# HiKapok/DAN

Hardware: AMD Instinct MI355X
Metric: 640x640 images/sec/node (train fwd+bwd) (higher is better)
Workload: dtype bf16; 1 GPU; S3FD VGG-16 backbone + 6 detection heads, 640x640 bf16 training (fwd+bwd+SGD), batch 16 per GPU; global_batch=16, parallelism=dp1, anchors_per_image=34125, step_launch=eager, rccl_ranks=1, weight_gradient_stream=True

## Files before the change

dan_amd/_lib.py:

```python
import ctypes
import os

import torch

_HERE = os.path.dirname(os.path.abspath(__file__))
ACT_NAME = os.environ.get("DANHIP_DTYPE", "bf16").lower()
if ACT_NAME not in ("bf16", "fp16"):
    raise ValueError("DANHIP_DTYPE must be bf16 or fp16, got %r" % ACT_NAME)
ACT_DTYPE = torch.float16 if ACT_NAME == "fp16" else torch.bfloat16
SO_PATH = os.path.join(_HERE, "libdanhip_f16.so" if ACT_NAME == "fp16" else "libdanhip.so")
if os.environ.get("DANHIP_LIB_PATH"):
    SO_PATH = os.path.abspath(os.environ["DANHIP_LIB_PATH"])

F32, BF16 = 0, 1
SPLIT3 = 3


class ConvDesc(ctypes.Structure):
    _fields_ = [(n, ctypes.c_int32) for n in ("N", "H", "W", "Cin", "Ho", "Wo", "Cout", "kh", "kw", "stride")]


class ConvPitch(ctypes.Structure):
    _fields_ = [(n, ctypes.c_int32) for n in ("x_pitch", "y_pitch", "aux_pitch")]


class PackEntry(ctypes.Structure):
    _fields_ = [("w_hwio", ctypes.c_void_p), ("wf_packed", ctypes.c_void_p), ("wb_packed", ctypes.c_void_p)] + \
               [(n, ctypes.c_int32) for n in ("kh", "kw", "cin", "cin_real", "cout", "rows_f", "cols_f", "rows_b", "cols_b", "co8", "first_block", "pad_")]


class JpegInfo(ctypes.Structure):
    _fields_ = [(n, ctypes.c_int32) for n in ("width", "height", "ncomp", "mode", "reason", "reserved")] + [("coef_count", ctypes.c_int64)]


class JpegDesc(ctypes.Structure):
    _fields_ = [(n, ctypes.c_int32) for n in ("width", "height", "ncomp", "mode")] + \
               [(n, ctypes.c_int32 * 3) for n in ("blocks_w", "blocks_h", "comp_w", "comp_h", "quant_index")] + \
               [(n, ctypes.c_int32) for n in ("status", "idct_groups", "rgb_groups")] + [("reserved", ctypes.c_int32 * 2)] + \
               [("coef_offset", ctypes.c_int64), ("coef_count", ctypes.c_int64), ("plane_offset", ctypes.c_int64 * 3),
                ("out_offset", ctypes.c_int64), ("quant", (ctypes.c_uint16 * 64) * 4)]


P = ctypes.c_void_p
I32 = ctypes.c_int32
I64 = ctypes.c_int64
FL = ctypes.c_float
DESC = ctypes.POINTER(ConvDesc)

SIGNATURES = {
    "danhip_conv_packed_dims": [DESC, ctypes.c_int, ctypes.POINTER(I64), ctypes.POINTER(I64)],
    "danhip_pack_conv_weight": [DESC, P, I32, P, P, P],
# ... 57 lines not shown
    "danhip_nms": [P, I32, I32, I32, FL, P, P, P],
    "danhip_argsort_desc_f32": [P, I64, I32, P, P, ctypes.c_size_t, P],
    "danhip_augment_preprocess": [P, I32, I32, I32, ctypes.POINTER(ctypes.c_int32), ctypes.POINTER(ctypes.c_float), I32, I32, I32, I32, I32, P, I32, I32,
                                  P, ctypes.c_size_t, P],
    "danhip_deform_psroi_pool_fwd": [P, P, P, P, P, I32, I32, I32, I32, I32, I32, I32, I32, I32, FL, FL, I32, I32, P],
    "danhip_deform_psroi_pool_bwd": [P, P, P, P, P, P, P, I32, I32, I32, I32, I32, I32, I32, I32, I32, I32, FL, FL, I32, I32, P],
    "danhip_maxpool3x3s2_same_fwd": [P, P, I32, I32, I32, I32, P],
    "danhip_maxpool3x3s2_same_bwd": [P, P, P, I32, I32, I32, I32, P],
    "danhip_resize_u8_linear": [P, I32, I32, P, I32, I32, I32, ctypes.c_double, ctypes.c_double, P],
    "danhip_bbox_vote": [P, P, I32, I32, ctypes.c_double, I32, P, P, P, ctypes.c_size_t, P],
    "danhip_wider_quantize": [P, ctypes.c_int, P, P, I32, I32, I32, P, P, I32, I32, P, P],
    "danhip_wider_score_range": [P, I64, P, P, ctypes.c_size_t, P],
    "danhip_wider_eval": [P, P, I64, P, P, P, I64, P, I32, I32, I32, I32, ctypes.c_double, P, ctypes.c_size_t, P, P],
    "danhip_wider_ap": [P, ctypes.c_size_t, P, I64, I32, I32, I32, P, P, P, P, P, P],
    "danhip_deform_sample_fwd": [P, P, P, I32, I32, I32, I32, I32, I32, I32, I32, I32, P],
    "danhip_deform_sample_bwd": [P, P, P, P, P, I32, I32, I32, I32, I32, I32, I32, I32, I32, ctypes.c_int, P, ctypes.c_size_t, P],
    "danhip_deform_conv_fwd": [P, P, P, P, P, I32, I32, I32, I32, I32, I32, I32, I32, I32, I32, ctypes.c_int, P, ctypes.c_size_t, P],
    "danhip_deform_conv_bwd": [P, P, P, P, P, P, P, P, I32, I32, I32, I32, I32, I32, I32, I32, I32, I32, ctypes.c_int, P, ctypes.c_size_t, P],
    "danhip_deform_conv_bwd_with_col": [P, P, P, P, P, P, P, P, P, I32, I32, I32, I32, I32, I32, I32, I32, I32, I32, ctypes.c_int, P, ctypes.c_size_t, P],
    "danhip_deform_conv_bwd_deliver": [P, P, P, P, P, P, P, P, P, I32, I32, I32, I32, I32, I32, I32, I32, I32, I32, ctypes.c_int, ctypes.c_int, P, ctypes.c_size_t, P],
    "danhip_cast_pad_f32_to_bf16": [P, P, P, I64, I32, I32, P],
    "danhip_head_split_fwd": [P, P, P, I32, I32, I32, I32, I32, I32, I32, P],
    "danhip_head_split_bwd": [P, P, P, P, I32, I32, I32, I32, I32, I32, I32, P],
    "danhip_hard_neg_select": [P, P, P, P, P, P, I32, I32, FL, ctypes.c_int, P],
    "danhip_detection_loss_fwd": [P, P, P, P, P, P, P, P, I32, I32, P],
    "danhip_detection_loss_bwd": [P, P, P, P, P, P, P, FL, FL, I32, I32, P],
    "danhip_sgd_momentum_flat": [P, P, P, P, P, P, I32, I64, FL, FL, FL, P, P],
    "danhip_sgd_momentum_flat_dynamic": [P, P, P, P, P, P, I32, I64, FL, FL, P, P, P],
    "danhip_anchors_generate": [P, P, P, P, P, P, I32, I32, I32, FL, FL, FL, I32, P],
    "danhip_iou_matrix": [P, P, P, P, P, P, P, I32, I32, P],
    "danhip_dual_max_match": [P, I32, I32, FL, FL, ctypes.c_int, P, P, P, ctypes.c_size_t, P],
    "danhip_small_mining_match": [P, I32, I32, FL, FL, FL, I32, FL, P, P, P, ctypes.c_size_t, P],
    "danhip_encode_anchors": [P, P, P, P, P, P, P, P, P, I32, FL, FL, FL, FL, FL, P],
    "danhip_decode_anchors": [P, P, P, P, P, P, I32, I32, FL, FL, FL, FL, P],
    "danhip_face_scores": [P, P, P, FL, I64, P],
    "danhip_comm_load": [ctypes.c_char_p],
    "danhip_comm_rccl_version": [ctypes.POINTER(ctypes.c_int)],
    "danhip_comm_unique_id": [P],
    "danhip_comm_create": [P, I32, I32, I32, ctypes.POINTER(ctypes.c_void_p)],
    "danhip_comm_destroy": [P],
    "danhip_comm_info": [P, ctypes.POINTER(I32), ctypes.POINTER(I32), ctypes.POINTER(I32)],
    "danhip_comm_async_error": [P, ctypes.POINTER(I32)],
    "danhip_comm_abort": [P],
    "danhip_comm_allreduce_sum": [P, P, I64, ctypes.c_int, P],
    "danhip_comm_reduce_scatter_sum": [P, P, P, I64, ctypes.c_int, P],
    "danhip_comm_allgather": [P, P, P, I64, ctypes.c_int, P],
# ... 139 lines not shown
```

dan_amd/csrc/capi.cpp:

```cpp
#include <cstdarg>
#include <cstdio>
#include <cstdlib>
#include <cstring>
#include <atomic>
#include <mutex>

#include <hip/hip_runtime.h>

#include "../../include/danhip.h"

static thread_local char g_err[512] = "";

void danhip_set_error(const char* fmt, ...) {
  va_list ap;
  va_start(ap, fmt);
  vsnprintf(g_err, sizeof(g_err), fmt, ap);
  va_end(ap);
}

extern "C" const char* danhip_last_error(void) { return g_err; }
extern "C" int danhip_version(void) { return 8; }
extern "C" int danhip_act_dtype(void) {
#ifdef DANHIP_FP16
  return DANHIP_F16;
#else
  return DANHIP_BF16;
#endif
}

namespace {
struct Opt { const char* name; const char* env; int def; std::atomic<int> value; };
Opt g_opts[] = {{"splitk", "DANHIP_SPLITK", 1, {0}}, {"wgrad_slab", "DANHIP_WGRAD_SLAB", 1, {0}}, {"halo_b2", "DANHIP_HALO_B2", 0, {0}},
                {"wgrad_b2", "DANHIP_WGRAD_B2", 0, {0}}, {"halo_general_epilogue", "DANHIP_HALO_GENERAL_EPILOGUE", 0, {0}},
                {"deform_bwd_form", "DANHIP_DEFORM_BWD_FORM", 0, {0}}, {"pw_dgrad_ld_bn", "DANHIP_PW_DGRAD_LD_BN", 128, {0}},
                {"wgrad_c8", "DANHIP_WGRAD_C8", 1, {0}}, {"deform_dx_untiled", "DANHIP_DEFORM_DX_UNTILED", 0, {0}}};
std::once_flag g_opts_once;
Opt* find_opt(const char* name) {
  std::call_once(g_opts_once, [] {
    for (Opt& o : g_opts) { const char* e = getenv(o.env); o.value.store(e ? atoi(e) : o.def, std::memory_order_relaxed); }
  });
  if (!name) return nullptr;
  for (Opt& o : g_opts)
    if (strcmp(o.name, name) == 0) return &o;
  return nullptr;
// ... 25 lines not shown
```

dan_amd/csrc/loss.hip:

```cpp
#include "common.h"

namespace {

__device__ __forceinline__ float block_sum(float v, float* sh) {
#pragma unroll
  for (int o = 32; o > 0; o >>= 1) v += __shfl_xor(v, o, 64);
  const int w = threadIdx.x >> 6, nw = blockDim.x >> 6;
  if ((threadIdx.x & 63) == 0) sh[w] = v;
  __syncthreads();
  float t = 0.f;
  for (int i = 0; i < nw; ++i) t += sh[i];
  __syncthreads();
  return t;
}

__global__ void head_split_fwd_kernel(const float* __restrict__ h, float* __restrict__ loc, float* __restrict__ cls, int B, int HW, int Ch,
                                      int nneg, int npos, int A, int off) {
  const long total = (long)B * HW;
  for (long m = (long)blockIdx.x * blockDim.x + threadIdx.x; m < total; m += (long)gridDim.x * blockDim.x) {
    const int b = (int)(m / HW), p = (int)(m % HW);
    const float* r = h + m * Ch;
    const long a = (long)b * A + off + p;
    *reinterpret_cast<float4*>(loc + a * 4) = make_float4(r[0], r[1], r[2], r[3]);
    float ng = r[4];
// ... 5 lines not shown
}

__global__ void head_split_bwd_kernel(const float* __restrict__ h, const float* __restrict__ dloc, const float* __restrict__ dcls,
                                      float* __restrict__ dy, int B, int HW, int Ch, int nneg, int npos, int A, int off) {
  const long total = (long)B * HW;
  for (long m = (long)blockIdx.x * blockDim.x + threadIdx.x; m < total; m += (long)gridDim.x * blockDim.x) {
    const int b = (int)(m / HW), p = (int)(m % HW);
    const float* r = h + m * Ch;
    const long a = (long)b * A + off + p;
    float* o = dy + m * Ch;
    for (int i = 0; i < 4; ++i) o[i] = dloc[a * 4 + i];
    for (int grp = 0; grp < 2; ++grp) {
      const int s = grp == 0 ? 4 : 4 + nneg, n = grp == 0 ? nneg : npos;
      float mx = r[s];
      for (int i = 1; i < n; ++i) mx = fmaxf(mx, r[s + i]);
      int cnt = 0;
      for (int i = 0; i < n; ++i) cnt += (r[s + i] == mx);
      const float g = dcls[a * 2 + grp] / (float)cnt;
      for (int i = 0; i < n; ++i) o[s + i] = r[s + i] == mx ? g : 0.f;
    }
  }
}

__global__ void hard_neg_scores_kernel(const float* __restrict__ cls, const int* __restrict__ labels, float* __restrict__ score,
                                       int* __restrict__ counts, int A) {
  __shared__ int sp, sn;
  if (threadIdx.x == 0) { sp = 0; sn = 0; }
  __syncthreads();
  const int b = blockIdx.y;
  int np = 0, nn = 0;
  for (int a = blockIdx.x * blockDim.x + threadIdx.x; a < A; a += gridDim.x * blockDim.x) {
    const long i = (long)b * A + a;
    const float2 l = *reinterpret_cast<const float2*>(cls + i * 2);
    const float mx = fmaxf(l.x, l.y);
    const float e0 = expf(l.x - mx), e1 = expf(l.y - mx);
    const float pbg = e0 / (e0 + e1);
    const int lab = labels[i];
    score[i] = lab == 0 ? 0.f - pbg : -1.f;
    np += lab > 0;
    nn += lab == 0;
  }
  atomicAdd(&sp, np);
  atomicAdd(&sn, nn);
  __syncthreads();
  if (threadIdx.x == 0) { atomicAdd(counts + b * 2, sp); atomicAdd(counts + b * 2 + 1, sn); }
}
// ... 200 lines not shown

extern "C" int danhip_head_split_fwd(const float* h, float* loc, float* cls, int32_t B, int32_t HW, int32_t Ch, int32_t nneg, int32_t npos,
                                     int32_t A, int32_t anchor_offset, void* stream) {
  DH_REQUIRE(h && loc && cls && B > 0 && HW > 0 && nneg >= 1 && npos >= 1 && Ch == 4 + nneg + npos, DANHIP_EINVAL,
             "head_split_fwd: bad arguments (Ch must be 4+nneg+npos, depth 1)");
  DH_REQUIRE(anchor_offset >= 0 && anchor_offset + HW <= A, DANHIP_EINVAL, "head_split_fwd: anchor range out of bounds");
  hipLaunchKernelGGL(head_split_fwd_kernel, dim3(grid_for((long)B * HW, 256)), dim3(256), 0, (hipStream_t)stream, h, loc, cls, B, HW, Ch, nneg,
                     npos, A, anchor_offset);
  DH_LAUNCH_CHECK();
  return DANHIP_OK;
}

extern "C" int danhip_head_split_bwd(const float* h, const float* dloc, const float* dcls, float* dy, int32_t B, int32_t HW, int32_t Ch,
                                     int32_t nneg, int32_t npos, int32_t A, int32_t anchor_offset, void* stream) {
  DH_REQUIRE(h && dloc && dcls && dy && B > 0 && HW > 0 && nneg >= 1 && npos >= 1 && Ch == 4 + nneg + npos, DANHIP_EINVAL,
             "head_split_bwd: bad arguments");
  DH_REQUIRE(anchor_offset >= 0 && anchor_offset + HW <= A, DANHIP_EINVAL, "head_split_bwd: anchor range out of bounds");
  hipLaunchKernelGGL(head_split_bwd_kernel, dim3(grid_for((long)B * HW, 256)), dim3(256), 0, (hipStream_t)stream, h, dloc, dcls, dy, B, HW, Ch,
                     nneg, npos, A, anchor_offset);
  DH_LAUNCH_CHECK();
  return DANHIP_OK;
}

extern "C" int danhip_hard_neg_select(const float* cls, const int32_t* labels, float* score, int32_t* counts, float* thr, int32_t* k_out,
                                      int32_t B, int32_t A, float negative_ratio, int at_least_one, void* stream) {
  DH_REQUIRE(cls && labels && score && counts && thr && k_out && B > 0 && A > 0, DANHIP_EINVAL, "hard_neg_select: bad arguments");
  hipStream_t s = (hipStream_t)stream;
  if (hipMemsetAsync(counts, 0, sizeof(int32_t) * 2 * B, s) != hipSuccess) { danhip_set_error("hard_neg_select: memset failed"); return DANHIP_ELAUNCH; }
  hipLaunchKernelGGL(hard_neg_scores_kernel, dim3((unsigned)grid_for(A, 1024, 8), (unsigned)B), dim3(1024), 0, s, cls, labels, score, counts, A);
  DH_LAUNCH_CHECK();
  if (A <= 36 * 1024)
    hipLaunchKernelGGL(kth_largest_rows_kernel<36>, dim3((unsigned)B), dim3(1024), 0, s, score, counts, thr, k_out, A, negative_ratio, at_least_one);
  else if (A <= 88 * 1024)
    hipLaunchKernelGGL(kth_largest_rows_kernel<88>, dim3((unsigned)B), dim3(1024), 0, s, score, counts, thr, k_out, A, negative_ratio, at_least_one);
  else
    hipLaunchKernelGGL(kth_largest_rows_kernel<0>, dim3((unsigned)B), dim3(1024), 0, s, score, counts, thr, k_out, A, negative_ratio, at_least_one);
  DH_LAUNCH_CHECK();
  return DANHIP_OK;
}

extern "C" int danhip_detection_loss_fwd(const float* cls, const float* loc, const int32_t* labels, const float* loc_targets, const float* score,
                                         const float* thr, uint8_t* sel, float* acc4, int32_t B, int32_t A, void* stream) {
  DH_REQUIRE(cls && loc && labels && loc_targets && score && thr && sel && acc4 && B > 0 && A > 0, DANHIP_EINVAL, "detection_loss_fwd: bad arguments");
  hipStream_t s = (hipStream_t)stream;
  if (hipMemsetAsync(acc4, 0, sizeof(float) * 4, s) != hipSuccess) { danhip_set_error("detection_loss_fwd: memset failed"); return DANHIP_ELAUNCH; }
  const long total = (long)B * A;
// ... 44 lines not shown
```

dan_amd/net/sfd_net.py:

```python
import os

import torch

from .. import ops
from .variables import VariableStore


POOL_ONLY = os.environ.get("DANHIP_POOL_ONLY", "1") == "1"


class VGG16Backbone(object):
    def __init__(self, data_format="channels_last", bn_epsilon=1e-5, bn_momentum=0.997, use_fused_bn=True, variables=None):
        if data_format != "channels_last":
            raise ValueError("the MI355X build is NHWC-native: use data_format='channels_last' "
                             "(the reference's eval scripts' default, eval_sfd.py:63)")
        self._data_format = data_format
        self._bn_epsilon = bn_epsilon
        self._bn_momentum = bn_momentum
        self._use_fused_bn = use_fused_bn
        self.vs = variables if variables is not None else VariableStore()

    def l2_normalize(self, inputs, init_value, training, name=None):
        w = self.vs.get((name or "l2_normalize") + "/weight", (inputs.shape[-1],), init_value)
        return ops.l2_normalize(inputs, w)
# ... 52 lines not shown
        inputs = self.conv_block(inputs, 2, 128, (3, 3), (1, 1), "conv2", pool_after=True, pool_only=POOL_ONLY)
        inputs = ops.max_pool_2x2(inputs)
        inputs = self.conv_block(inputs, 3, 256, (3, 3), (1, 1), "conv3", pool_after=True)
        feature_layers.append(self.l2_normalize(tap(inputs), 10, training, "l2_norm_layer_3"))
        inputs = ops.max_pool_2x2(inputs)
        inputs = self.conv_block(inputs, 3, 512, (3, 3), (1, 1), "conv4", pool_after=True)
        feature_layers.append(self.l2_normalize(tap(inputs), 8, training, "l2_norm_layer_4"))
        inputs = ops.max_pool_2x2(inputs)
        inputs = self.conv_block(inputs, 3, 512, (3, 3), (1, 1), "conv5", pool_after=True)
        feature_layers.append(self.l2_normalize(tap(inputs), 5, training, "l2_norm_layer_5"))
        inputs = ops.max_pool_2x2(inputs)
        inputs = self.conv_relu(inputs, 1024, (3, 3), (1, 1), "fc6")
        inputs = self.conv_relu(inputs, 1024, (1, 1), (1, 1), "fc7")
        feature_layers.append(tap(inputs))
        inputs = self.conv_relu(inputs, 256, (1, 1), (1, 1), "additional_layers/conv6_1")
        inputs = self.conv_relu(inputs, 512, (3, 3), (2, 2), "additional_layers/conv6_2")
        feature_layers.append(tap(inputs))
        inputs = self.conv_relu(inputs, 128, (1, 1), (1, 1), "additional_layers/conv7_1")
        inputs = self.conv_relu(inputs, 256, (3, 3), (2, 2), "additional_layers/conv7_2")
        feature_layers.append(tap(inputs))
        return feature_layers

    def predict_heads(self, feature_layers, pos_maxout, neg_maxout, num_anchors_depth_per_layer, name, shared_conv=False):
        B = feature_layers[0].shape[0]
        assert all(d == 1 for d in num_anchors_depth_per_layer), "one anchor per cell (all reference configs)"
        A = sum(f.shape[1] * f.shape[2] for f in feature_layers)
        dev = feature_layers[0].device
        loc = torch.zeros((B, A, 4), dtype=torch.float32, device=dev)
        cls = torch.zeros((B, A, 2), dtype=torch.float32, device=dev)
        off = 0
        for ind, feat in enumerate(feature_layers):
            if shared_conv:
                feat = self.conv_relu(feat, feat.shape[-1], (3, 3), (1, 1), "{}/shared_conv_{}".format(name, ind))
            c = feat.shape[-1]
            ncls = pos_maxout[ind] + neg_maxout[ind]
            wl = self.vs.get("{}/loc_{}/kernel".format(name, ind), (3, 3, c, 4), "glorot")
            bl = self.vs.get("{}/loc_{}/bias".format(name, ind), (4,), "zeros")
            wc = self.vs.get("{}/cls_{}/kernel".format(name, ind), (3, 3, c, ncls), "glorot")
            bc = self.vs.get("{}/cls_{}/bias".format(name, ind), (ncls,), "zeros")
            pre = "{}/loc_{}/".format(name, ind), "{}/cls_{}/".format(name, ind)
            wf = self.vs.fuse((pre[0] + "kernel", pre[1] + "kernel"), axis=3)
            bf = self.vs.fuse((pre[0] + "bias", pre[1] + "bias"), axis=0)
            if wf is None or bf is None:
                wf, bf = ops.cat_static([wl, wc], 3), ops.cat_static([bl, bc], 0)
            h = ops.conv2d(feat, wf, bf, stride=1, relu=False, out_f32=True)
            if ops.TRACE is not None and ncls > 2:
                ops.TRACE.setdefault("maxout", {})[id(wc)] = h.detach()[..., 4:]
            loc, cls = ops.head_split(h, loc, cls, neg_maxout[ind], pos_maxout[ind], off)
            off += feat.shape[1] * feat.shape[2]
        return loc, cls

    def multibox_head(self, feature_layers, pos_maxout, neg_maxout, num_anchors_depth_per_layer):
        return self.predict_heads(feature_layers, pos_maxout, neg_maxout, num_anchors_depth_per_layer, "multibox_head")


import contextlib


@contextlib.contextmanager
def precision_scope(precision):
    ctx = ops.context()
    prev = ctx.SPLIT_EVAL
    ctx.SPLIT_EVAL = precision == "split"
    if precision == "split":
        ops.split_range_reset()
    try:
        yield
    finally:
        ctx.SPLIT_EVAL = prev
    if precision == "split":
        ops.split_range_check()


# ... 7 lines not shown
```

dan_amd/ops.py:

```python
import contextlib
import ctypes
import os

import torch

from . import _lib
from ._lib import ACT_DTYPE as ACT, BF16, F32, SPLIT3, ConvDesc, call, ptr, stream


class OpsContext(object):
    __slots__ = ("USE_SPLITK", "USE_SLOTS", "USE_RELU_BITS", "USE_POOL_ARG", "USE_JUNCTION", "POOL_ONLY_TRAIN", "KEEP_DEFORM_COL", "WGRAD_STREAM", "WGRAD_FIRST", "FUSE_FIRST_WGRAD", "SPLIT_EVAL", "TRACE",
                 "PROFILE", "PROFILE_BYTES", "GRAD_READY_HOOK", "LOSS_SCALE_DEV", "wgrad")

    def __init__(self, **overrides):
        env = os.environ.get
        self.USE_SPLITK = True
        self.USE_SLOTS = True
        self.USE_RELU_BITS = env("DANHIP_RELU_BITS", "1") == "1"
        self.USE_POOL_ARG = env("DANHIP_POOL_ARG", "1") == "1"
        self.USE_JUNCTION = env("DANHIP_JUNCTION", "1") == "1"
        self.POOL_ONLY_TRAIN = env("DANHIP_POOL_ONLY_TRAIN", "1") == "1"
        self.KEEP_DEFORM_COL = True
        self.WGRAD_STREAM = env("DANHIP_WGRAD_STREAM", "1") == "1"
        self.WGRAD_FIRST = env("DANHIP_WGRAD_FIRST", "0") == "1"
        self.FUSE_FIRST_WGRAD = env("DANHIP_FUSE_FIRST_WGRAD", "1") == "1"
        self.SPLIT_EVAL = False
        self.TRACE = self.PROFILE = self.PROFILE_BYTES = None
        self.GRAD_READY_HOOK = self.LOSS_SCALE_DEV = None
        self.wgrad = {"on": False, "side": None, "main": None, "keep": []}
        for k, v in overrides.items():
            setattr(self, k, v)


_CTX = OpsContext()
_CTX_FIELDS = frozenset(OpsContext.__slots__) - {"wgrad"}


def context():
    return _CTX


@contextlib.contextmanager
def use_context(ctx):
    global _CTX
    prev, _CTX = _CTX, ctx
    try:
        yield ctx
    finally:
# ... 331 lines not shown
                parg = _pool_arg_buffer(pooled, need_bwd and tracked)
                pool_out.extend([pooled, parg])
            call("danhip_conv2d_fwd_relu_bits_arg", ctypes.byref(d), ptr(x), ptr(wf), ptr(b.detach()), yp, ptr(ybits), ptr(pooled), ptr(pbits), ptr(parg),
                 stream())
            bits_out.extend([ybits, pbits])
        elif pool_out is not None:
            assert relu and not out_f32 and residual is None and b is not None and cout % 8 == 0
            pooled = torch.empty((N, (d.Ho + 1) // 2, (d.Wo + 1) // 2, cout), dtype=ACT, device=x.device)
            parg = _pool_arg_buffer(pooled, need_bwd and tracked)
            ws, nws = _conv_scratch(d, 0, x.device)
            if nws:
                assert not skip_y
                call("danhip_conv2d_fwd_ws", ctypes.byref(d), ptr(x), ptr(wf), ptr(b.detach()), ptr(y), BF16, 1, None, ptr(ws), nws, stream())
                call("danhip_maxpool2x2_fwd_arg", ptr(y), ptr(pooled), ptr(parg), N, d.Ho, d.Wo, cout, stream())
            else:
                call("danhip_conv2d_fwd_pool_arg", ctypes.byref(d), ptr(x), ptr(wf), ptr(b.detach()), yp, ptr(pooled), ptr(parg), stream())
            pool_out.extend([pooled, parg])
        else:
            ws, nws = _conv_scratch(d, 0, x.device)
            call("danhip_conv2d_fwd_ws", ctypes.byref(d), ptr(x), ptr(wf), ptr(b.detach()) if b is not None else None, ptr(y),
                 F32 if out_f32 else BF16, int(relu), ptr(residual), ptr(ws), nws, stream())
        _prof_end(e0, d, 4 if pool_out is not None else 0, wrote_y=not skip_y, pooled=pool_out is not None)
        ctx.d, ctx.relu, ctx.cin_real = d, relu, cin_real
        ctx.xslot, ctx.yslot, ctx.xbits = xslot, yslot, xbits
        ctx.set_materialize_grads(False)
        ctx.has_res = residual is not None
        ctx.w_param, ctx.b_param = w_param, b_param
        ctx.save_for_backward(x, wb, y if (relu and not skip_y) else None)
        ctx.y_unwritten = skip_y
        ctx.has_bias = b is not None
        ctx.block_w, ctx.block_b = bool(block_grads & 1), bool(block_grads & 2)
        return y

    @staticmethod
    def backward(ctx, dy):
        x, wb, y = ctx.saved_tensors
        d = ctx.d
        co8 = (d.Cout + 7) // 8 * 8
        M = d.N * d.Ho * d.Wo
        wp, bp = ctx.w_param, ctx.b_param
        need_dw = ctx.needs_input_grad[1] or ctx.block_w
        need_db = ctx.has_bias and (ctx.needs_input_grad[2] or ctx.block_b)
        db_sink = _grad_sink(bp) if bp is not None else None
        db = None
        if need_db:
            db = db_sink if db_sink is not None else torch.zeros(d.Cout, dtype=torch.float32, device=x.device)
# ... 1 lines not shown
        dres = None
        if dy is not None and ctx.y_unwritten:
            raise RuntimeError("conv2d(pool_only=True): the full-resolution activation was never written, but a gradient reached it outside the "
                               "fused pool's direct hand-off (some op other than max_pool_2x2 consumed it)")
        if dy is not None:
            if ctx.has_res:
                dres = dy
            if dy.dtype != ACT or dy.shape[-1] != co8:
                src = dy.contiguous().to(torch.float32)
                dyp = torch.empty((d.N, d.Ho, d.Wo, co8), dtype=ACT, device=dy.device)
                call("danhip_cast_pad_f32_to_bf16", ptr(src), ptr(y) if (ctx.relu and d.Cout != co8) else None, ptr(dyp), M, d.Cout, co8, stream())
                dy, owned = dyp, True
                masked = ctx.relu and d.Cout != co8
            else:
                dy, owned = dy.contiguous(), False
                masked = False
            if ctx.relu and not masked:
                if not owned:
                    dy = dy.clone()
                call("danhip_relu_bwd_bias_grad", ptr(dy), ptr(y), None, M, co8, stream())
            g = dy if g is None else g.add_(dy)
        if g is None:
            return (None,) * 19
        db_in_wgrad = need_db and need_dw
        if need_db and not db_in_wgrad:
            if co8 == d.Cout:
                call("danhip_relu_bwd_bias_grad", ptr(g), None, ptr(db), M, co8, stream())
            else:
                db.add_(g.view(M, co8)[:, :d.Cout].to(torch.float32).sum(0))
        dx = None
        dw = None
        hooked = False
        fused_first = False

        def launch_dx():
            nonlocal dx, fused_first
            if ctx.needs_input_grad[0]:
                xs = ctx.xslot
                fi = ctx.first
                if (fi is not None and _CTX.FUSE_FIRST_WGRAD and xs is not None and xs.is_relu and xs.count == 0 and ctx.xbits is not None
                        and _grad_sink(fi[1]) is not None and (fi[2] is None or _grad_sink(fi[2]) is not None)
                        and _lib.lib().danhip_conv2d_bwd_data_first_supported(ctypes.byref(d))):
                    e0 = _prof_begin()
                    call("danhip_conv2d_bwd_data_bits_first", ctypes.byref(d), ptr(g), ptr(wb), ptr(relu_bits(x, ctx.xbits)), ptr(fi[0]), int(fi[3]),
                         ptr(_grad_sink(fi[1])), ptr(_grad_sink(fi[2])) if fi[2] is not None else None, stream())
                    _prof_end(e0, d, 5, wrote_y=False)
# ... 236 lines not shown
                               None if residual is None else residual[i:i + nmax], padding, want_f32=True) for i in range(0, N, nmax)]
        return torch.cat(parts, dim=0)
    xe = _limb_exp(x) if _is_limbs(x) else LIMB_EXP
    x3 = split3(x, xe)
    d3 = _desc(N, H, W, x3.shape[-1], cout, kh, kw, stride, padding == "valid")
    wf, we = _split_weight(d3, w, cin)
    limbs = not want_f32 and residual is None and cout % 8 == 0 and N * d3.Ho * d3.Wo * 3 * cout < (1 << 31)
    if limbs:
        y = torch.empty((N, d3.Ho, d3.Wo, 3 * cout), dtype=torch.float16, device=x.device)
    else:
        y = torch.empty((N, d3.Ho, d3.Wo, cout), dtype=torch.float32, device=x.device)
    n = _lib.lib_f16().danhip_conv2d_workspace_bytes(ctypes.byref(d3), 0) if -(-(N * d3.Ho * d3.Wo) // 128) * -(-cout // 128) <= 160 else 0
    ws = torch.empty(n, dtype=torch.uint8, device=x.device) if n else None
    ye = LIMB_EXP if limbs else 0
    _lib.call_f16("danhip_conv2d_fwd_split", ctypes.byref(d3), ptr(x3), ptr(wf), ptr(_split_bias(b, ye)) if b is not None else None, ptr(y),
                  SPLIT3 if limbs else F32, int(relu), xe - we - ye, ptr(ws), n, stream())
    if limbs:
        return _limb_view(y, cout, LIMB_EXP)
    if residual is not None:
        y.add_(_f32_in(residual))
    return y


def conv2d(x, w, b=None, stride=1, relu=False, out_f32=False, residual=None, pool=False, padding="same", pool_only=False):
    if _is_limbs(x) or (_CTX.SPLIT_EVAL and _f32_infer(x)):
        return _conv2d_split(x, w, b, stride, relu, residual, padding, want_f32=out_f32)
    if _f32_infer(x):
        return _conv2d_f32(x, w, b, stride, relu, _f32_in(residual), padding)
    wp = w if (isinstance(w, torch.nn.Parameter) or hasattr(w, "_danhip_grad")) else None
    bp = b if (isinstance(b, torch.nn.Parameter) or hasattr(b, "_danhip_grad")) else None
    track = torch.is_grad_enabled() and (x.requires_grad or w.requires_grad or _sink_trainable(w))
    if track and relu and residual is not None:
        raise NotImplementedError("relu + fused residual needs a separate ReLU mask in backward (y > 0 is not the mask)")
    yslot = _new_slot(track and not out_f32)
    pool_out = [] if (pool and relu and not out_f32 and residual is None and b is not None and w.shape[-1] % 8 == 0) else None
    if padding not in ("same", "valid"):
        raise ValueError("padding must be 'same' or 'valid'")
    blk = 0
    if torch.is_grad_enabled():
        blk = (1 if _sink_trainable(w) else 0) | (2 if (b is not None and _sink_trainable(b)) else 0)
    xs = _slot_of(x) if track else None
    xbits = _bits_holder(x) if (xs is not None and xs.is_relu and _CTX.USE_RELU_BITS) else None
    bits_out = [] if (track and relu and _CTX.USE_RELU_BITS) else None
    po = (1 if not track else (2 if (_CTX.POOL_ONLY_TRAIN and _CTX.TRACE is None and _CTX.USE_SLOTS and yslot is not None) else 0)) if pool_only else 0
    y = _Conv2d.apply(x, w, b, stride, relu, out_f32, residual, wp, bp, xs, yslot, pool_out, padding == "valid", blk, xbits, bits_out,
                      po, bool(track), getattr(x, "_dh_first", None) if track else None)
    if (track and relu and not x.requires_grad and wp is not None and x.shape[-1] == 8 and w.shape[2] <= 4 and w.shape[3] == 64 and w.shape[0] == 3
            and w.shape[1] == 3 and stride == 1 and padding == "same" and residual is None and not out_f32):
        y._dh_first = (x, wp, bp, w.shape[2])
    if getattr(y, "_dh_already_pooled", False):
        return y
    if _CTX.TRACE is not None and relu and wp is not None:
        _CTX.TRACE[id(wp)] = y.detach()
    if bits_out:
        y._dh_bits = [bits_out[0]]
    if yslot is not None:
        cout = w.shape[-1]
        if cout % 8 == 0:
            yslot.__init__(y, relu)
            y._dh_slot = yslot
        else:
            yslot.__init__(y, relu, (cout + 7) // 8 * 8)
            y._dh_pslot = yslot
    if pool_out:
        y._dh_pooled = pool_out[0]
        y._dh_pool_arg = pool_out[1]
        if bits_out and bits_out[1] is not None:
            y._dh_pooled_bits = bits_out[1]
    return y


class _MaxPool(torch.autograd.Function):

    @staticmethod
    def forward(ctx, x, xslot, yslot, pre=None, arg=None):
        N, H, W, C = x.shape
        if pre is not None:
            y = pre
        else:
# ... 181 lines not shown

    @staticmethod
    def forward(ctx, h, loc, cls, nneg, npos, off):
        B, H, W, Ch = h.shape
        A = loc.shape[1]
        call("danhip_head_split_fwd", ptr(h), ptr(loc), ptr(cls), B, H * W, Ch, nneg, npos, A, off, stream())
        ctx.save_for_backward(h)
        ctx.cfg = (nneg, npos, off, A)
        ctx.mark_dirty(loc, cls)
        return loc, cls

    @staticmethod
    def backward(ctx, dloc, dcls):
        (h,) = ctx.saved_tensors
        nneg, npos, off, A = ctx.cfg
        B, H, W, Ch = h.shape
        dy = torch.empty((B, H, W, Ch), dtype=torch.float32, device=h.device)
        call("danhip_head_split_bwd", ptr(h), ptr(dloc.contiguous()), ptr(dcls.contiguous()), ptr(dy), B, H * W, Ch, nneg, npos, A, off, stream())
        return dy, dloc, dcls, None, None, None


def head_split(h, loc, cls, nneg, npos, off):
    return _HeadSplit.apply(h, loc, cls, nneg, npos, off)




class _DetectionLoss(torch.autograd.Function):

    @staticmethod
    def forward(ctx, cls, loc, labels, loc_t, ratio, at_least_one, scale):
        B, A, _ = cls.shape
        assert cls.dtype == torch.float32 and loc.dtype == torch.float32 and loc_t.dtype == torch.float32, "detection_loss: fp32 logits / targets"
        assert labels.dtype == torch.int32 and labels.shape == (B, A), "detection_loss: labels must be int32 [B, A]"
        assert cls.is_contiguous() and loc.is_contiguous() and labels.is_contiguous() and loc_t.is_contiguous()
        dev = cls.device
        score = torch.empty((B, A), dtype=torch.float32, device=dev)
        counts = torch.empty((B, 2), dtype=torch.int32, device=dev)
        thr = torch.empty((B,), dtype=torch.float32, device=dev)
        k = torch.empty((B,), dtype=torch.int32, device=dev)
        sel = torch.empty((B, A), dtype=torch.uint8, device=dev)
        acc = torch.empty((4,), dtype=torch.float32, device=dev)
        call("danhip_hard_neg_select", ptr(cls), ptr(labels), ptr(score), ptr(counts), ptr(thr), ptr(k), B, A, float(ratio), int(at_least_one), stream())
        call("danhip_detection_loss_fwd", ptr(cls), ptr(loc), ptr(labels), ptr(loc_t), ptr(score), ptr(thr), ptr(sel), ptr(acc), B, A, stream())
        if _CTX.TRACE is not None:
            _CTX.TRACE.setdefault("loss_sel", []).append(sel)
# ... 760 lines not shown
```

include/danhip.h:

```cpp
#ifndef DANHIP_H_
#define DANHIP_H_
#include <stddef.h>
#include <stdint.h>

#ifdef __cplusplus
extern "C" {
#endif

#define DANHIP_OK 0
#define DANHIP_EINVAL (-1)
#define DANHIP_ELAUNCH (-2)
#define DANHIP_EWORKSPACE (-3)

#define DANHIP_F32 0
#define DANHIP_BF16 1
#define DANHIP_F16 2
#define DANHIP_SPLIT3 3

const char* danhip_last_error(void);
int danhip_version(void);
int danhip_set_option(const char* name, int value);
int danhip_get_option(const char* name);
int danhip_act_dtype(void);

// ... 94 lines not shown
int danhip_residual_bwd(const uint16_t* dy, const uint16_t* r, const uint16_t* x_mask, uint16_t* dr, uint16_t* dx, int accumulate, int64_t n,
                        void* stream);
int danhip_avgpool2x2s1_same_fwd_strided(const uint16_t* x, int32_t x_pitch, uint16_t* y, int32_t y_pitch, int32_t N, int32_t H, int32_t W,
                                         int32_t C, int relu, void* stream);
int danhip_avgpool2x2s1_same_bwd_strided(const uint16_t* dy, int32_t y_pitch, uint16_t* dx, int32_t x_pitch, int32_t N, int32_t H, int32_t W,
                                         int32_t C, void* stream);
int danhip_slice_deliver(const uint16_t* dy, int32_t ldy, int32_t c0, int32_t C, const uint16_t* mask, int32_t ldm, uint16_t* out, int32_t Cpad,
                         int accumulate, int64_t M, void* stream);
int danhip_batchnorm_fwd_train(const uint16_t* x, const float* gamma, const float* beta, uint16_t* y, float* save_mean,
                               float* save_rstd, float* moving_mean, float* moving_var, int64_t M, int32_t C, float eps,
                               float momentum, int relu, float* workspace, void* stream);
int danhip_batchnorm_fwd_infer(const uint16_t* x, const float* gamma, const float* beta, const float* mean, const float* rstd,
                               uint16_t* y, int64_t M, int32_t C, int relu, void* stream);
int danhip_batchnorm_bwd(const uint16_t* x, const uint16_t* dy, const float* gamma, const float* save_mean, const float* save_rstd,
                         uint16_t* dx, float* dgamma, float* dbeta, int64_t M, int32_t C, void* stream);
int danhip_preprocess_u8(const uint8_t* img_rgb, uint16_t* out, int64_t npix, void* stream);
int danhip_cast_pad_f32_to_bf16(const float* src, const uint16_t* relu_y, uint16_t* dst, int64_t rows, int32_t c_src, int32_t c_dst,
                                void* stream);

int danhip_head_split_fwd(const float* h, float* loc, float* cls, int32_t B, int32_t HW, int32_t Ch, int32_t nneg, int32_t npos,
                          int32_t A, int32_t anchor_offset, void* stream);
int danhip_head_split_bwd(const float* h, const float* dloc, const float* dcls, float* dy, int32_t B, int32_t HW, int32_t Ch,
                          int32_t nneg, int32_t npos, int32_t A, int32_t anchor_offset, void* stream);
int danhip_hard_neg_select(const float* cls, const int32_t* labels, float* score, int32_t* counts, float* thr, int32_t* k_out,
                           int32_t B, int32_t A, float negative_ratio, int at_least_one, void* stream);
int danhip_detection_loss_fwd(const float* cls, const float* loc, const int32_t* labels, const float* loc_targets,
                              const float* score, const float* thr, uint8_t* sel, float* acc4, int32_t B, int32_t A,
                              void* stream);
int danhip_detection_loss_bwd(const float* cls, const float* loc, const float* loc_targets, const uint8_t* sel,
                              const float* acc4, float* dcls, float* dloc, float ce_scale, float loc_scale, int32_t B,
                              int32_t A, void* stream);
int danhip_sgd_momentum_flat(float* w, const float* g, float* v, const int64_t* seg_starts, const float* gmult,
                             const float* wd_coef, int32_t nseg, int64_t total, float lr, float momentum, float grad_scale,
                             float* l2_out, void* stream);
int danhip_sgd_momentum_flat_dynamic(float* w, const float* g, float* v, const int64_t* seg_starts, const float* gmult,
                                     const float* wd_coef, int32_t nseg, int64_t total, float lr, float momentum,
                                     float* loss_scale_state, float* l2_out, void* stream);

int danhip_anchors_generate(float* ymin, float* xmin, float* ymax, float* xmax, const float* anchor_h, const float* anchor_w,
                            int32_t depth, int32_t layer_h, int32_t layer_w, float stride, float offset_h, float offset_w,
                            int32_t out_offset, void* stream);
int danhip_iou_matrix(const float* ymin, const float* xmin, const float* ymax, const float* xmax, const uint8_t* inside_mask,
                      const float* gt_boxes, float* overlaps, int32_t A, int32_t G, void* stream);
size_t danhip_match_workspace_bytes(int32_t A, int32_t G);
int danhip_dual_max_match(const float* overlaps, int32_t A, int32_t G, float low_thres, float high_thres, int ignore_between,
                          int32_t* match_indices, float* match_scores, void* workspace, size_t workspace_bytes, void* stream);
// ... 223 lines not shown
```

Baseline: 1309 images/sec.

## Batch all detection-head splits into one kernel and write padded bf16 dY slots directly

Forward replaces six per-level head_split calls, each of which updated torch.zeros loc/cls buffers, with one kernel that walks a per-level table and writes loc/cls into empty buffers. Backward fuses the maxout gradient routing, the bf16 cast and the channel padding into one kernel that writes straight into each head conv's dY slot. This drops several small launches, the zero-fills and the separate fp32 dY plus cast/pad passes. The cost is a more involved slot protocol (hslot), an 8-level limit and alignment requirements, with a fallback to the old per-level path.

```diff
diff --git a/dan_amd/_lib.py b/dan_amd/_lib.py
--- a/dan_amd/_lib.py
+++ b/dan_amd/_lib.py
@@ -27,6 +27,13 @@
 class PackEntry(ctypes.Structure):
     _fields_ = [("w_hwio", ctypes.c_void_p), ("wf_packed", ctypes.c_void_p), ("wb_packed", ctypes.c_void_p)] + \
                [(n, ctypes.c_int32) for n in ("kh", "kw", "cin", "cin_real", "cout", "rows_f", "cols_f", "rows_b", "cols_b", "co8", "first_block", "pad_")]
+
+
+HEADS_MAX_LEVELS = 8
+
+
+class HeadLevel(ctypes.Structure):
+    _fields_ = [("h", ctypes.c_void_p), ("dy", ctypes.c_void_p)] + [(n, ctypes.c_int32) for n in ("HW", "Ch", "nneg", "npos", "off", "co_pad")]
 
 
 class JpegInfo(ctypes.Structure):
@@ -130,6 +137,8 @@
     "danhip_cast_pad_f32_to_bf16": [P, P, P, I64, I32, I32, P],
     "danhip_head_split_fwd": [P, P, P, I32, I32, I32, I32, I32, I32, I32, P],
     "danhip_head_split_bwd": [P, P, P, P, I32, I32, I32, I32, I32, I32, I32, P],
+    "danhip_heads_split_fwd": [ctypes.POINTER(HeadLevel), I32, P, P, I32, I32, P],
+    "danhip_heads_grad_pad": [ctypes.POINTER(HeadLevel), I32, P, P, I32, I32, P],
     "danhip_hard_neg_select": [P, P, P, P, P, P, I32, I32, FL, ctypes.c_int, P],
     "danhip_detection_loss_fwd": [P, P, P, P, P, P, P, P, I32, I32, P],
     "danhip_detection_loss_bwd": [P, P, P, P, P, P, P, FL, FL, I32, I32, P],
diff --git a/dan_amd/csrc/capi.cpp b/dan_amd/csrc/capi.cpp
--- a/dan_amd/csrc/capi.cpp
+++ b/dan_amd/csrc/capi.cpp
@@ -19,7 +19,7 @@
 }
 
 extern "C" const char* danhip_last_error(void) { return g_err; }
-extern "C" int danhip_version(void) { return 8; }
+extern "C" int danhip_version(void) { return 9; }
 extern "C" int danhip_act_dtype(void) {
 #ifdef DANHIP_FP16
   return DANHIP_F16;
diff --git a/dan_amd/csrc/loss.hip b/dan_amd/csrc/loss.hip
--- a/dan_amd/csrc/loss.hip
+++ b/dan_amd/csrc/loss.hip
@@ -51,6 +51,119 @@
   }
 }
 
+struct HeadsTable {
+  const float* h[DANHIP_HEADS_MAX_LEVELS];
+  bf16_t* dy[DANHIP_HEADS_MAX_LEVELS];
+  long row0[DANHIP_HEADS_MAX_LEVELS + 1];
+  int HW[DANHIP_HEADS_MAX_LEVELS], Ch[DANHIP_HEADS_MAX_LEVELS], nneg[DANHIP_HEADS_MAX_LEVELS], off[DANHIP_HEADS_MAX_LEVELS],
+      co_pad[DANHIP_HEADS_MAX_LEVELS];
+  int n;
+};
+
+__global__ void heads_split_fwd_kernel(const HeadsTable t, float* __restrict__ loc, float* __restrict__ cls, int A) {
+  const long total = t.row0[t.n];
+  for (long m = (long)blockIdx.x * blockDim.x + threadIdx.x; m < total; m += (long)gridDim.x * blockDim.x) {
+    int l = 0;
+    while (l + 1 < t.n && m >= t.row0[l + 1]) ++l;
+    const long ml = m - t.row0[l];
+    const int HW = t.HW[l], Ch = t.Ch[l], nneg = t.nneg[l], npos = Ch - 4 - nneg;
+    const int b = (int)(ml / HW), p = (int)(ml % HW);
+    const float* r = t.h[l] + ml * Ch;
+    const long a = (long)b * A + t.off[l] + p;
+    *reinterpret_cast<float4*>(loc + a * 4) = make_float4(r[0], r[1], r[2], r[3]);
+    float ng = r[4];
+    for (int i = 1; i < nneg; ++i) ng = fmaxf(ng, r[4 + i]);
+    float ps = r[4 + nneg];
+    for (int i = 1; i < npos; ++i) ps = fmaxf(ps, r[4 + nneg + i]);
+    *reinterpret_cast<float2*>(cls + a * 2) = make_float2(ng, ps);
+  }
+}
+
+__device__ __forceinline__ uint4 pack8_rne(const float* f) {
+  uint4 o;
+  o.x = (unsigned)f2bf(f[0]) | ((unsigned)f2bf(f[1]) << 16);
+  o.y = (unsigned)f2bf(f[2]) | ((unsigned)f2bf(f[3]) << 16);
+  o.z = (unsigned)f2bf(f[4]) | ((unsigned)f2bf(f[5]) << 16);
+  o.w = (unsigned)f2bf(f[6]) | ((unsigned)f2bf(f[7]) << 16);
+  return o;
+}
+
+__global__ void heads_grad_pad_kernel(const HeadsTable t, const float* __restrict__ dloc, const float* __restrict__ dcls, int A) {
+  const long total = t.row0[t.n];
+  for (long m = (long)blockIdx.x * blockDim.x + threadIdx.x; m < total; m += (long)gridDim.x * blockDim.x) {
+    int l = 0;
+    while (l + 1 < t.n && m >= t.row0[l + 1]) ++l;
+    const long ml = m - t.row0[l];
+    const int HW = t.HW[l], Ch = t.Ch[l], nneg = t.nneg[l], co_pad = t.co_pad[l];
+    const int b = (int)(ml / HW), p = (int)(ml % HW);
+    const float* r = t.h[l] + ml * Ch;
+    const long a = (long)b * A + t.off[l] + p;
+    const float4 dl = *reinterpret_cast<const float4*>(dloc + a * 4);
+    const float2 dc = *reinterpret_cast<const float2*>(dcls + a * 2);
+    uint4* o = reinterpret_cast<uint4*>(t.dy[l] + ml * co_pad);
+    const int pos0 = 4 + nneg;
+    if (Ch <= 8) {
+      float v[8];
+      if (Ch == 8) {
+        const float4 lo = reinterpret_cast<const float4*>(r)[0], hi = reinterpret_cast<const float4*>(r)[1];
+        v[0] = lo.x; v[1] = lo.y; v[2] = lo.z; v[3] = lo.w; v[4] = hi.x; v[5] = hi.y; v[6] = hi.z; v[7] = hi.w;
+      } else if (Ch == 6) {
+        const float2 c0 = reinterpret_cast<const float2*>(r)[0], c1 = reinterpret_cast<const float2*>(r)[1], c2 = reinterpret_cast<const float2*>(r)[2];
+        v[0] = c0.x; v[1] = c0.y; v[2] = c1.x; v[3] = c1.y; v[4] = c2.x; v[5] = c2.y; v[6] = 0.f; v[7] = 0.f;
+      } else {
+#pragma unroll
+        for (int i = 0; i < 8; ++i) v[i] = i < Ch ? r[i] : 0.f;
+      }
+      float mxn = v[4], mxp = 0.f;
+#pragma unroll
+      for (int j = 5; j < 8; ++j) {
+        if (j < pos0) mxn = fmaxf(mxn, v[j]);
+        else if (j == pos0) mxp = v[j];
+        else if (j < Ch) mxp = fmaxf(mxp, v[j]);
+      }
+      int cn = 0, cp = 0;
+#pragma unroll
+      for (int j = 4; j < 8; ++j) {
+        if (j < pos0) cn += (v[j] == mxn);
+        else if (j < Ch) cp += (v[j] == mxp);
+      }
+      const float gn = dc.x / (float)cn, gp = dc.y / (float)cp;
+      float g[8] = {dl.x, dl.y, dl.z, dl.w, 0.f, 0.f, 0.f, 0.f};
+#pragma unroll
+      for (int j = 4; j < 8; ++j) {
+        if (j < pos0) g[j] = v[j] == mxn ? gn : 0.f;
+        else if (j < Ch) g[j] = v[j] == mxp ? gp : 0.f;
+      }
+      o[0] = pack8_rne(g);
+      for (int c = 8; c < co_pad; c += 8) o[c >> 3] = make_uint4(0u, 0u, 0u, 0u);
+    } else {
+      float mx[2], gg[2];
+      for (int grp = 0; grp < 2; ++grp) {
+        const int s = grp == 0 ? 4 : pos0, n = grp == 0 ? nneg : Ch - pos0;
+        float q = r[s];
+        for (int i = 1; i < n; ++i) q = fmaxf(q, r[s + i]);
+        int cnt = 0;
+        for (int i = 0; i < n; ++i) cnt += (r[s + i] == q);
+        mx[grp] = q;
+        gg[grp] = (grp == 0 ? dc.x : dc.y) / (float)cnt;
+      }
+      for (int c = 0; c < co_pad; c += 8) {
+        float g[8];
+#pragma unroll
+        for (int k = 0; k < 8; ++k) {
+          const int j = c + k;
+          float x = 0.f;
+          if (j < 4) x = j == 0 ? dl.x : j == 1 ? dl.y : j == 2 ? dl.z : dl.w;
+          else if (j < pos0) x = r[j] == mx[0] ? gg[0] : 0.f;
+          else if (j < Ch) x = r[j] == mx[1] ? gg[1] : 0.f;
+          g[k] = x;
+        }
+        o[c >> 3] = pack8_rne(g);
+      }
+    }
+  }
+}
+
 __global__ void hard_neg_scores_kernel(const float* __restrict__ cls, const int* __restrict__ labels, float* __restrict__ score,
                                        int* __restrict__ counts, int A) {
   __shared__ int sp, sn;
@@ -297,6 +410,66 @@
   return DANHIP_OK;
 }
 
+static int heads_table(const danhip_head_level* lv, int32_t n, int32_t B, int32_t A, bool grad, const char* who, HeadsTable* t) {
+  DH_REQUIRE(lv && B > 0 && A > 0, DANHIP_EINVAL, "%s: bad arguments", who);
+  DH_REQUIRE(n >= 1 && n <= DANHIP_HEADS_MAX_LEVELS, DANHIP_EINVAL, "%s: %d levels (1 .. %d fit the table)", who, n, DANHIP_HEADS_MAX_LEVELS);
+  int order[DANHIP_HEADS_MAX_LEVELS];
+  t->n = n;
+  t->row0[0] = 0;
+  for (int l = 0; l < n; ++l) {
+    const danhip_head_level& e = lv[l];
+    DH_REQUIRE(e.h && (!grad || e.dy), DANHIP_EINVAL, "%s: level %d: null pointer", who, l);
+    DH_REQUIRE(((uintptr_t)e.h & 15) == 0 && (!grad || ((uintptr_t)e.dy & 15) == 0), DANHIP_EINVAL, "%s: level %d: pointers must be 16-byte aligned", who, l);
+    DH_REQUIRE(e.HW > 0 && e.nneg >= 1 && e.npos >= 1 && e.Ch == 4 + e.nneg + e.npos, DANHIP_EINVAL,
+               "%s: level %d: Ch=%d must be 4 + nneg + npos (nneg=%d, npos=%d, depth 1)", who, l, e.Ch, e.nneg, e.npos);
+    DH_REQUIRE(!grad || (e.co_pad >= e.Ch && e.co_pad % 8 == 0), DANHIP_EINVAL, "%s: level %d: co_pad=%d must be a multiple of 8 and >= Ch=%d", who, l,
+               e.co_pad, e.Ch);
+    DH_REQUIRE(e.off >= 0 && (long)e.off + e.HW <= A, DANHIP_EINVAL, "%s: level %d: anchor range [%d, %ld) outside [0, %d)", who, l, e.off,
+               (long)e.off + e.HW, A);
+    t->h[l] = e.h; t->dy[l] = grad ? e.dy : nullptr;
+    t->HW[l] = e.HW; t->Ch[l] = e.Ch; t->nneg[l] = e.nneg; t->off[l] = e.off; t->co_pad[l] = grad ? e.co_pad : 0;
+    t->row0[l + 1] = t->row0[l] + (long)B * e.HW;
+    int i = l;
+    for (; i > 0 && lv[order[i - 1]].off > e.off; --i) order[i] = order[i - 1];
+    order[i] = l;
+  }
+  long next = 0;
+  for (int i = 0; i < n; ++i) {
+    DH_REQUIRE(lv[order[i]].off == next, DANHIP_EINVAL, "%s: the levels' anchor ranges must tile [0, %d) without gap or overlap (level %d starts at %d, expected %ld)",
+               who, A, order[i], lv[order[i]].off, next);
+    next += lv[order[i]].HW;
+  }
+  DH_REQUIRE(next == A, DANHIP_EINVAL, "%s: the levels' anchor ranges end at %ld, not at A=%d", who, next, A);
+  for (int l = n; l < DANHIP_HEADS_MAX_LEVELS; ++l) {
+    t->h[l] = nullptr; t->dy[l] = nullptr; t->HW[l] = 1; t->Ch[l] = 0; t->nneg[l] = 0; t->off[l] = 0; t->co_pad[l] = 0;
+    t->row0[l + 1] = t->row0[n];
+  }
+  return DANHIP_OK;
+}
+
+extern "C" int danhip_heads_split_fwd(const danhip_head_level* levels, int32_t nlevels, float* loc, float* cls, int32_t B, int32_t A, void* stream) {
+  DH_REQUIRE(loc && cls && ((uintptr_t)loc & 15) == 0 && ((uintptr_t)cls & 7) == 0, DANHIP_EINVAL,
+             "heads_split_fwd: loc / cls must be non-null and 16- / 8-byte aligned");
+  HeadsTable t;
+  if (int rc = heads_table(levels, nlevels, B, A, false, "heads_split_fwd", &t)) return rc;
+  const long rows = t.row0[t.n];
+  hipLaunchKernelGGL(heads_split_fwd_kernel, dim3(grid_for(rows, 256)), dim3(256), 0, (hipStream_t)stream, t, loc, cls, A);
+  DH_LAUNCH_CHECK();
+  return DANHIP_OK;
+}
+
+extern "C" int danhip_heads_grad_pad(const danhip_head_level* levels, int32_t nlevels, const float* dloc, const float* dcls, int32_t B, int32_t A,
+                                     void* stream) {
+  DH_REQUIRE(dloc && dcls && ((uintptr_t)dloc & 15) == 0 && ((uintptr_t)dcls & 7) == 0, DANHIP_EINVAL,
+             "heads_grad_pad: dloc / dcls must be non-null and 16- / 8-byte aligned");
+  HeadsTable t;
+  if (int rc = heads_table(levels, nlevels, B, A, true, "heads_grad_pad", &t)) return rc;
+  const long rows = t.row0[t.n];
+  hipLaunchKernelGGL(heads_grad_pad_kernel, dim3(grid_for(rows, 256)), dim3(256), 0, (hipStream_t)stream, t, dloc, dcls, A);
+  DH_LAUNCH_CHECK();
+  return DANHIP_OK;
+}
+
 extern "C" int danhip_hard_neg_select(const float* cls, const int32_t* labels, float* score, int32_t* counts, float* thr, int32_t* k_out,
                                       int32_t B, int32_t A, float negative_ratio, int at_least_one, void* stream) {
   DH_REQUIRE(cls && labels && score && counts && thr && k_out && B > 0 && A > 0, DANHIP_EINVAL, "hard_neg_select: bad arguments");
diff --git a/dan_amd/net/sfd_net.py b/dan_amd/net/sfd_net.py
--- a/dan_amd/net/sfd_net.py
+++ b/dan_amd/net/sfd_net.py
@@ -98,13 +98,8 @@
         return feature_layers
 
     def predict_heads(self, feature_layers, pos_maxout, neg_maxout, num_anchors_depth_per_layer, name, shared_conv=False):
-        B = feature_layers[0].shape[0]
         assert all(d == 1 for d in num_anchors_depth_per_layer), "one anchor per cell (all reference configs)"
-        A = sum(f.shape[1] * f.shape[2] for f in feature_layers)
-        dev = feature_layers[0].device
-        loc = torch.zeros((B, A, 4), dtype=torch.float32, device=dev)
-        cls = torch.zeros((B, A, 2), dtype=torch.float32, device=dev)
-        off = 0
+        hs = []
         for ind, feat in enumerate(feature_layers):
             if shared_conv:
                 feat = self.conv_relu(feat, feat.shape[-1], (3, 3), (1, 1), "{}/shared_conv_{}".format(name, ind))
@@ -119,12 +114,11 @@
             bf = self.vs.fuse((pre[0] + "bias", pre[1] + "bias"), axis=0)
             if wf is None or bf is None:
                 wf, bf = ops.cat_static([wl, wc], 3), ops.cat_static([bl, bc], 0)
-            h = ops.conv2d(feat, wf, bf, stride=1, relu=False, out_f32=True)
+            h = ops.conv2d(feat, wf, bf, stride=1, relu=False, out_f32=True, dy_slot=ops.context().HEADS_BATCHED)
             if ops.TRACE is not None and ncls > 2:
                 ops.TRACE.setdefault("maxout", {})[id(wc)] = h.detach()[..., 4:]
-            loc, cls = ops.head_split(h, loc, cls, neg_maxout[ind], pos_maxout[ind], off)
-            off += feat.shape[1] * feat.shape[2]
-        return loc, cls
+            hs.append(h)
+        return ops.heads_split(hs, list(zip(neg_maxout, pos_maxout)))
 
     def multibox_head(self, feature_layers, pos_maxout, neg_maxout, num_anchors_depth_per_layer):
         return self.predict_heads(feature_layers, pos_maxout, neg_maxout, num_anchors_depth_per_layer, "multibox_head")
diff --git a/dan_amd/ops.py b/dan_amd/ops.py
--- a/dan_amd/ops.py
+++ b/dan_amd/ops.py
@@ -9,7 +9,7 @@
 
 
 class OpsContext(object):
-    __slots__ = ("USE_SPLITK", "USE_SLOTS", "USE_RELU_BITS", "USE_POOL_ARG", "USE_JUNCTION", "POOL_ONLY_TRAIN", "KEEP_DEFORM_COL", "WGRAD_STREAM", "WGRAD_FIRST", "FUSE_FIRST_WGRAD", "SPLIT_EVAL", "TRACE",
+    __slots__ = ("USE_SPLITK", "USE_SLOTS", "USE_RELU_BITS", "USE_POOL_ARG", "USE_JUNCTION", "POOL_ONLY_TRAIN", "KEEP_DEFORM_COL", "WGRAD_STREAM", "WGRAD_FIRST", "FUSE_FIRST_WGRAD", "HEADS_BATCHED", "SPLIT_EVAL", "TRACE",
                  "PROFILE", "PROFILE_BYTES", "GRAD_READY_HOOK", "LOSS_SCALE_DEV", "wgrad")
 
     def __init__(self, **overrides):
@@ -24,6 +24,7 @@
         self.WGRAD_STREAM = env("DANHIP_WGRAD_STREAM", "1") == "1"
         self.WGRAD_FIRST = env("DANHIP_WGRAD_FIRST", "0") == "1"
         self.FUSE_FIRST_WGRAD = env("DANHIP_FUSE_FIRST_WGRAD", "1") == "1"
+        self.HEADS_BATCHED = env("DANHIP_HEADS_BATCHED", "1") == "1"
         self.SPLIT_EVAL = False
         self.TRACE = self.PROFILE = self.PROFILE_BYTES = None
         self.GRAD_READY_HOOK = self.LOSS_SCALE_DEV = None
@@ -401,6 +402,7 @@
                  F32 if out_f32 else BF16, int(relu), ptr(residual), ptr(ws), nws, stream())
         _prof_end(e0, d, 4 if pool_out is not None else 0, wrote_y=not skip_y, pooled=pool_out is not None)
         ctx.d, ctx.relu, ctx.cin_real = d, relu, cin_real
+        ctx.out_f32 = out_f32
         ctx.xslot, ctx.yslot, ctx.xbits = xslot, yslot, xbits
         ctx.set_materialize_grads(False)
         ctx.has_res = residual is not None
@@ -448,6 +450,8 @@
             g = dy if g is None else g.add_(dy)
         if g is None:
             return (None,) * 19
+        if _CTX.TRACE is not None and ctx.out_f32:
+            _CTX.TRACE.setdefault("head_dy", []).append(g)
         db_in_wgrad = need_db and need_dw
         if need_db and not db_in_wgrad:
             if co8 == d.Cout:
@@ -730,7 +734,7 @@
     return y
 
 
-def conv2d(x, w, b=None, stride=1, relu=False, out_f32=False, residual=None, pool=False, padding="same", pool_only=False):
+def conv2d(x, w, b=None, stride=1, relu=False, out_f32=False, residual=None, pool=False, padding="same", pool_only=False, dy_slot=False):
     if _is_limbs(x) or (_CTX.SPLIT_EVAL and _f32_infer(x)):
         return _conv2d_split(x, w, b, stride, relu, residual, padding, want_f32=out_f32)
     if _f32_infer(x):
@@ -741,6 +745,9 @@
     if track and relu and residual is not None:
         raise NotImplementedError("relu + fused residual needs a separate ReLU mask in backward (y > 0 is not the mask)")
     yslot = _new_slot(track and not out_f32)
+    hslot = None
+    if dy_slot and out_f32 and not relu and residual is None:
+        yslot = hslot = _new_slot(track)
     pool_out = [] if (pool and relu and not out_f32 and residual is None and b is not None and w.shape[-1] % 8 == 0) else None
     if padding not in ("same", "valid"):
         raise ValueError("padding must be 'same' or 'valid'")
@@ -762,7 +769,11 @@
         _CTX.TRACE[id(wp)] = y.detach()
     if bits_out:
         y._dh_bits = [bits_out[0]]
-    if yslot is not None:
+    if hslot is not None:
+        hslot.__init__(y, False, (w.shape[-1] + 7) // 8 * 8)
+        hslot.dtype = ACT
+        y._dh_hslot = hslot
+    elif yslot is not None:
         cout = w.shape[-1]
         if cout % 8 == 0:
             yslot.__init__(y, relu)
@@ -990,6 +1001,61 @@
 
 def head_split(h, loc, cls, nneg, npos, off):
     return _HeadSplit.apply(h, loc, cls, nneg, npos, off)
+
+
+class _HeadsSplit(torch.autograd.Function):
+
+    @staticmethod
+    def forward(ctx, cfg, slots, *hs):
+        B = hs[0].shape[0]
+        levels = (_lib.HeadLevel * len(hs))()
+        off = 0
+        for e, h, (nneg, npos) in zip(levels, hs, cfg):
+            assert h.dtype == torch.float32 and h.is_contiguous() and h.dim() == 4 and h.shape[0] == B, "heads_split: fp32 NHWC head maps of one batch"
+            e.h, e.dy = h.data_ptr(), None
+            e.HW, e.Ch, e.nneg, e.npos, e.off, e.co_pad = h.shape[1] * h.shape[2], h.shape[3], nneg, npos, off, 0
+            off += e.HW
+        loc = torch.empty((B, off, 4), dtype=torch.float32, device=hs[0].device)
+        cls = torch.empty((B, off, 2), dtype=torch.float32, device=hs[0].device)
+        call("danhip_heads_split_fwd", levels, len(hs), ptr(loc), ptr(cls), B, off, stream())
+        ctx.save_for_backward(*hs)
+        ctx.levels, ctx.slots, ctx.dims = levels, slots, (B, off)
+        return loc, cls
+
+    @staticmethod
+    def backward(ctx, dloc, dcls):
+        hs = ctx.saved_tensors
+        B, A = ctx.dims
+        assert dloc.dtype == torch.float32 and dcls.dtype == torch.float32 and dloc.shape == (B, A, 4) and dcls.shape == (B, A, 2)
+        dloc, dcls = dloc.contiguous(), dcls.contiguous()
+        if dloc.data_ptr() % 16:
+            dloc = dloc.clone()
+        if dcls.data_ptr() % 8:
+            dcls = dcls.clone()
+        levels = ctx.levels
+        for e, h, slot in zip(levels, hs, ctx.slots):
+            buf, acc = slot.target()
+            if acc:
+                raise RuntimeError("heads_split: a head convolution's dY slot was filled before the heads' backward ran")
+            e.h, e.dy, e.co_pad = h.data_ptr(), buf.data_ptr(), buf.shape[-1]
+        call("danhip_heads_grad_pad", levels, len(hs), ptr(dloc), ptr(dcls), B, A, stream())
+        return (None, None) + (None,) * len(hs)
+
+
+def heads_split(hs, cfg):
+    track = torch.is_grad_enabled() and any(h.requires_grad for h in hs)
+    slots = [getattr(h, "_dh_hslot", None) for h in hs]
+    if _CTX.HEADS_BATCHED and len(hs) <= _lib.HEADS_MAX_LEVELS and (not track or all(s is not None for s in slots)):
+        return _HeadsSplit.apply([tuple(c) for c in cfg], slots, *hs)
+    B, dev = hs[0].shape[0], hs[0].device
+    A = sum(h.shape[1] * h.shape[2] for h in hs)
+    loc = torch.zeros((B, A, 4), dtype=torch.float32, device=dev)
+    cls = torch.zeros((B, A, 2), dtype=torch.float32, device=dev)
+    off = 0
+    for h, (nneg, npos) in zip(hs, cfg):
+        loc, cls = head_split(h, loc, cls, nneg, npos, off)
+        off += h.shape[1] * h.shape[2]
+    return loc, cls
 
 
 
diff --git a/include/danhip.h b/include/danhip.h
--- a/include/danhip.h
+++ b/include/danhip.h
@@ -140,6 +140,17 @@
                           int32_t A, int32_t anchor_offset, void* stream);
 int danhip_head_split_bwd(const float* h, const float* dloc, const float* dcls, float* dy, int32_t B, int32_t HW, int32_t Ch,
                           int32_t nneg, int32_t npos, int32_t A, int32_t anchor_offset, void* stream);
+#define DANHIP_HEADS_MAX_LEVELS 8
+typedef struct danhip_head_level {
+  const float* h;
+  uint16_t* dy;
+  int32_t HW, Ch, nneg, npos;
+  int32_t off;
+  int32_t co_pad;
+} danhip_head_level;
+int danhip_heads_split_fwd(const danhip_head_level* levels, int32_t nlevels, float* loc, float* cls, int32_t B, int32_t A, void* stream);
+int danhip_heads_grad_pad(const danhip_head_level* levels, int32_t nlevels, const float* dloc, const float* dcls, int32_t B, int32_t A,
+                          void* stream);
 int danhip_hard_neg_select(const float* cls, const int32_t* labels, float* score, int32_t* counts, float* thr, int32_t* k_out,
                            int32_t B, int32_t A, float negative_ratio, int at_least_one, void* stream);
 int danhip_detection_loss_fwd(const float* cls, const float* loc, const int32_t* labels, const float* loc_targets,
```

Result: faster. 1323 images/sec (median of 6 runs) (+1.0%).
